# zombie-einstein/bourse

Hardware: AMD Instinct MI355X
Metric: book-steps/sec (higher is better)
Workload: dtype u32

## Files before the change

bourse_amd/csrc/event_asm.hpp:

```cpp
#pragma once
#include <hip/hip_runtime.h>
#include <stdint.h>

namespace bkd {

#define EA_BIT "s[40:41]"
#define EA_C0 "s[42:43]"
#define EA_C1 "s[44:45]"
#define EA_E0 "s[46:47]"
#define EA_E1 "s[48:49]"
#define EA_EW "s50"
#define EA_P "s51"
#define EA_V "s52"
#define EA_ID "s53"
#define EA_KK "s54"
#define EA_BEST "s55"
#define EA_PV "s56"
#define EA_PID "s57"
#define EA_TV "s58"
#define EA_LS "s59"
#define EA_X "s60"
#define EA_X2 "s61"

#define EA_IF2_1(x) ""
#define EA_IF2_2(x) x
#define EA_IF1_1(x) x
#define EA_IF1_2(x) ""

#define EA_DPP(OP)                                                                                \
  "s_nop 1\n\t" OP " %[vm], %[vm], %[vm] quad_perm:[1,0,3,2] row_mask:0xf bank_mask:0xf\n\t"      \
  "s_nop 1\n\t" OP " %[vm], %[vm], %[vm] quad_perm:[2,3,0,1] row_mask:0xf bank_mask:0xf\n\t"      \
  "s_nop 1\n\t" OP " %[vm], %[vm], %[vm] row_half_mirror row_mask:0xf bank_mask:0xf\n\t"          \
  "s_nop 1\n\t" OP " %[vm], %[vm], %[vm] row_mirror row_mask:0xf bank_mask:0xf\n\t"               \
  "s_nop 1\n\t" OP " %[vm], %[vm], %[vm] row_bcast:15 row_mask:0xa bank_mask:0xf\n\t"             \
  "s_nop 1\n\t" OP " %[vm], %[vm], %[vm] row_bcast:31 row_mask:0xc bank_mask:0xf\n\t"             \
  "s_nop 1\n\t"

#define EA_LOOP(PH, KEND)                       \
  "s_add_u32 %[k], %[k], 1\n\t"                 \
  "s_cmp_lt_u32 %[k], " KEND "\n\t"             \
  "s_cbranch_scc1 L_top_" PH "_%=\n\t"          \
  "s_branch L_end_" PH "_%=\n\t"

#define EA_PICK(Q, EQ, L)                                              \
  "s_ff1_i32_b64 " EA_LS ", " EQ "\n\t"                                \
  "v_readlane_b32 " EA_PV ", %[vol" Q "], " EA_LS "\n\t"               \
  "v_readlane_b32 " EA_PID ", %[id" Q "], " EA_LS "\n\t"               \
  "s_mov_b32 m0, " EA_LS "\n\t"                                        \
  "s_min_u32 " EA_TV ", " EA_V ", " EA_PV "\n\t"                       \
  "s_sub_u32 " EA_PV ", " EA_PV ", " EA_TV "\n\t"                      \
  "v_writelane_b32 %[vol" Q "], " EA_PV ", m0\n\t"                     \
  "s_cmp_lg_u32 " EA_PV ", 0\n\t"                                      \
  "s_cbranch_scc1 L_trade_" L "\n\t"                                   \
  "s_andn2_b64 %[live" Q "], %[live" Q "], " EQ "\n\t"

#ifndef BOURSE_AMD_ASM_ALWAYS_TIE
#define BOURSE_AMD_ASM_ALWAYS_TIE 0
#endif
#if BOURSE_AMD_ASM_ALWAYS_TIE
#define EA_TIE_TEST(L, NR) ""
#else
#define EA_TIE_TEST(L, NR)                                                                 \
  "s_bcnt1_i32_b64 " EA_X ", " EA_E0 "\n\t"                                                \
  EA_IF2_##NR("s_bcnt1_i32_b64 " EA_X2 ", " EA_E1 "\n\t"                                   \
              "s_add_u32 " EA_X ", " EA_X ", " EA_X2 "\n\t")                               \
  "s_cmp_eq_u32 " EA_X ", 1\n\t"                                                           \
  "s_cbranch_scc1 L_pick_" L "\n\t"
#endif

#define EA_SIDE(L, PH, KEND, RG, NR, CAND, SENT, VOP, DOP, NOX, KKI)                                     \
  KKI "\n\t"                                                                                        \
  "s_and_b32 " EA_X ", " EA_V ", %[tmask]\n\t"           \
  "s_cbranch_scc0 L_rest_" L "\n\t"                                                                 \
  "L_match_" L ":\n\t"                                                                              \
  CAND " " EA_C0 ", %[live0], %[bid0]\n\t"                      \
  EA_IF2_##NR(CAND " " EA_C1 ", %[live1], %[bid1]\n\t"                                              \
              "s_or_b64 " EA_E0 ", " EA_C0 ", " EA_C1 "\n\t")                                       \
  "s_cbranch_scc0 L_rest_" L "\n\t"                                   \
  "v_cndmask_b32_e64 %[vm], " SENT ", %[price0], " EA_C0 "\n\t"                                     \
  EA_IF2_##NR("v_cndmask_b32_e64 %[vm2], " SENT ", %[price1], " EA_C1 "\n\t"                        \
              VOP " %[vm], %[vm], %[vm2]\n\t")                                                      \
  EA_DPP(DOP)                                                                                       \
  "v_readlane_b32 " EA_BEST ", %[vm], 63\n\t"                                                       \
  NOX " " EA_P ", " EA_BEST "\n\t"                                                                  \
  "s_cbranch_scc1 L_rest_" L "\n\t"                                                                 \
  "v_cmp_eq_u32_e64 " EA_E0 ", " EA_BEST ", %[price0]\n\t"                                          \
  EA_IF2_##NR("v_cmp_eq_u32_e64 " EA_E1 ", " EA_BEST ", %[price1]\n\t")                             \
  "s_and_b64 " EA_E0 ", " EA_E0 ", " EA_C0 "\n\t"                                                   \
  EA_IF2_##NR("s_and_b64 " EA_E1 ", " EA_E1 ", " EA_C1 "\n\t")                                      \
  EA_TIE_TEST(L, NR)                                                                                \
   \
  "v_cndmask_b32_e64 %[vm], -1, %[seq0], " EA_E0 "\n\t"                                             \
  EA_IF2_##NR("v_cndmask_b32_e64 %[vm2], -1, %[seq1], " EA_E1 "\n\t"                                \
              "v_min_u32 %[vm], %[vm], %[vm2]\n\t")                                                 \
  EA_DPP("v_min_u32_dpp")                                                                           \
  "v_readlane_b32 " EA_X ", %[vm], 63\n\t"                                                          \
  "s_nop 1\n\t"                                                                                     \
  "v_cmp_eq_u32_e64 " EA_C0 ", " EA_X ", %[seq0]\n\t"                                               \
  EA_IF2_##NR("v_cmp_eq_u32_e64 " EA_C1 ", " EA_X ", %[seq1]\n\t")                                  \
  "s_and_b64 " EA_E0 ", " EA_E0 ", " EA_C0 "\n\t"                                                   \
  EA_IF2_##NR("s_and_b64 " EA_E1 ", " EA_E1 ", " EA_C1 "\n\t")                                      \
  "L_pick_" L ":\n\t"                                                                               \
  EA_IF2_##NR("s_cmp_lg_u64 " EA_E0 ", 0\n\t"                                                       \
              "s_cbranch_scc0 L_pick1_" L "\n\t")                                                   \
  EA_PICK("0", EA_E0, L)                                                                            \
  EA_IF2_##NR("s_branch L_trade_" L "\n\t"                                                          \
              "L_pick1_" L ":\n\t"                                                                  \
              EA_PICK("1", EA_E1, L))                                                               \
  "L_trade_" L ":\n\t"                                   \
  "s_sub_u32 " EA_V ", " EA_V ", " EA_TV "\n\t"                                                     \
  "s_add_u32 %[tvol], %[tvol], " EA_TV "\n\t"                                                       \
  "s_mov_b32 m0, %[trn]\n\t"                                                                        \
  "v_writelane_b32 %[trk], " EA_KK ", m0\n\t"                                                       \
  "v_writelane_b32 %[trp], " EA_BEST ", m0\n\t"                                                     \
  "v_writelane_b32 %[trv], " EA_TV ", m0\n\t"                                                       \
  "v_writelane_b32 %[tra], " EA_ID ", m0\n\t"                                                       \
  "v_writelane_b32 %[trs], " EA_PID ", m0\n\t"                                                      \
  "s_add_u32 %[trn], %[trn], 1\n\t"                                                                 \
  "s_cmp_eq_u32 %[trn], 64\n\t"                                                                     \
  "s_cbranch_scc1 L_full_" L "\n\t"                                                                 \
  "s_cmp_lg_u32 " EA_V ", 0\n\t"                                                                    \
  "s_cbranch_scc1 L_match_" L "\n\t"                                                                \
  EA_LOOP(PH, KEND)                                                      \
  "L_full_" L ":\n\t"                                               \
  "s_cmp_eq_u32 " EA_V ", 0\n\t"                                                                    \
  "s_cbranch_scc1 L_fullnext_%=\n\t"                                                                \
  "s_mov_b32 m0, " EA_EW "\n\t"                                                                     \
  "v_writelane_b32 %[vol" RG "], " EA_V ", m0\n\t"        \
  "s_branch L_flush_%=\n\t"                                                                         \
  "L_rest_" L ":\n\t"                                                                               \
  "s_cmp_eq_u32 " EA_P ", " SENT "\n\t"                   \
  "s_cbranch_scc1 L_next_" PH "_%=\n\t"                                                             \
  "s_mov_b32 m0, " EA_EW "\n\t"                                                                     \
  "v_writelane_b32 %[vol" RG "], " EA_V ", m0\n\t"                                                  \
  "v_writelane_b32 %[seq" RG "], %[seqc], m0\n\t"                                                   \
  "s_lshl_b64 " EA_BIT ", 1, " EA_EW "\n\t"                                                         \
  "s_or_b64 %[live" RG "], %[live" RG "], " EA_BIT "\n\t"                                           \
  "s_add_u32 %[seqc], %[seqc], 1\n\t"                                                               \
  EA_LOOP(PH, KEND)

#define EA_NEW(PH, KEND, RG, NR)                                                                          \
  "v_readlane_b32 " EA_P ", %[price" RG "], " EA_EW "\n\t"                                          \
  "v_readlane_b32 " EA_V ", %[vol" RG "], " EA_EW "\n\t"                                            \
  "v_readlane_b32 " EA_ID ", %[id" RG "], " EA_EW "\n\t"                                            \
  "s_bitcmp1_b32 " EA_EW ", 14\n\t"                                                                 \
  "s_cbranch_scc1 L_bid_" PH RG "_%=\n\t"                                                           \
  EA_SIDE("a" PH RG "_%=", PH, KEND, RG, NR, "s_and_b64", "0", "v_max_u32", "v_max_u32_dpp", "s_cmp_gt_u32", \
          "s_or_b32 " EA_KK ", %[k], 0x80000000")                                                   \
  "L_bid_" PH RG "_%=:\n\t"                                                                         \
  EA_SIDE("b" PH RG "_%=", PH, KEND, RG, NR, "s_andn2_b64", "-1", "v_min_u32", "v_min_u32_dpp", "s_cmp_lt_u32", \
          "s_mov_b32 " EA_KK ", %[k]")

#define EA_PHASE(PH, KEND, NR)                                                                      \
  "L_top_" PH "_%=:\n\t"                                                                            \
  "v_readlane_b32 " EA_EW ", %[ev" PH "], %[k]\n\t"                                                 \
  "s_bitcmp1_b32 " EA_EW ", 15\n\t"                                                                 \
  "s_cbranch_scc1 L_new_" PH "_%=\n\t"                                                              \
  "s_lshl_b64 " EA_BIT ", 1, " EA_EW "\n\t"                                       \
  EA_IF2_##NR("s_bitcmp1_b32 " EA_EW ", 6\n\t"                                                      \
              "s_cbranch_scc1 L_can1_" PH "_%=\n\t")                                                \
  "s_andn2_b64 %[live0], %[live0], " EA_BIT "\n\t"                                                  \
  EA_IF2_##NR(EA_LOOP(PH, KEND)                                                                     \
              "L_can1_" PH "_%=:\n\t"                                                               \
              "s_andn2_b64 %[live1], %[live1], " EA_BIT "\n\t")                                     \
  "L_next_" PH "_%=:\n\t"                                                                           \
  EA_LOOP(PH, KEND)                                                                                 \
  "L_new_" PH "_%=:\n\t"                                                                            \
  EA_IF2_##NR("s_bitcmp1_b32 " EA_EW ", 6\n\t"                                                      \
              "s_cbranch_scc1 L_new1_" PH "_%=\n\t")                                                \
  EA_IF1_##NR("s_nop 1\n\t")                                \
  EA_NEW(PH, KEND, "0", NR)                                                                               \
  EA_IF2_##NR("L_new1_" PH "_%=:\n\t"                                                               \
              EA_NEW(PH, KEND, "1", NR))

__device__ __forceinline__ uint32_t events_asm_r2(uint32_t& k, uint32_t n_ev, uint32_t tmask, uint32_t& tr_n,
                                                  uint32_t& seq_ctr, uint32_t& trade_vol, uint64_t& live0,
                                                  uint64_t& live1, uint64_t bid0, uint64_t bid1, uint32_t price0,
                                                  uint32_t price1, uint32_t& vol0, uint32_t& vol1, uint32_t id0,
                                                  uint32_t id1, uint32_t& seq0, uint32_t& seq1, uint32_t ev0,
                                                  uint32_t ev1, uint32_t& trk, uint32_t& trp, uint32_t& trv,
                                                  uint32_t& tra, uint32_t& trs) {
  uint32_t st, vm, vm2;
  auto u32 = [](uint32_t x) { return (uint32_t)__builtin_amdgcn_readfirstlane(x); };
  auto u64 = [&](uint64_t x) { return ((uint64_t)u32((uint32_t)(x >> 32)) << 32) | u32((uint32_t)x); };
  k = u32(k);
  n_ev = u32(n_ev);
  tmask = u32(tmask);
  tr_n = u32(tr_n);
  seq_ctr = u32(seq_ctr);
  trade_vol = u32(trade_vol);
  live0 = u64(live0);
  live1 = u64(live1);
  bid0 = u64(bid0);
  bid1 = u64(bid1);
  const uint32_t kend0 = n_ev < 64u ? n_ev : 64u;
  asm volatile(
      "s_cmp_lt_u32 %[k], %[kend0]\n\t"
      "s_cbranch_scc1 L_top_0_%=\n\t"
      "s_branch L_end_0_%=\n\t"
      EA_PHASE("0", "%[kend0]", 2)
      "L_end_0_%=:\n\t"
      "s_cmp_lt_u32 %[k], %[nev]\n\t"
      "s_cbranch_scc0 L_done_%=\n\t"
      EA_PHASE("1", "%[nev]", 2)
      "L_end_1_%=:\n\t"
      "L_done_%=:\n\t"
      "s_mov_b32 %[st], 0\n\t"
      "s_branch L_out_%=\n\t"
      "L_fullnext_%=:\n\t"
      "s_add_u32 %[k], %[k], 1\n\t"
      "L_flush_%=:\n\t"
      "s_mov_b32 %[st], 1\n\t"
      "L_out_%=:\n\t"
      "s_nop 1"
      : [st] "=&s"(st), [vm] "=&v"(vm), [vm2] "=&v"(vm2), [k] "+s"(k), [trn] "+s"(tr_n), [seqc] "+s"(seq_ctr),
        [tvol] "+s"(trade_vol), [live0] "+s"(live0), [live1] "+s"(live1), [vol0] "+v"(vol0), [vol1] "+v"(vol1),
        [seq0] "+v"(seq0), [seq1] "+v"(seq1), [trk] "+v"(trk), [trp] "+v"(trp), [trv] "+v"(trv), [tra] "+v"(tra),
        [trs] "+v"(trs)
      : [price0] "v"(price0), [price1] "v"(price1), [id0] "v"(id0), [id1] "v"(id1), [ev0] "v"(ev0), [ev1] "v"(ev1),
        [bid0] "s"(bid0), [bid1] "s"(bid1), [nev] "s"(n_ev), [kend0] "s"(kend0), [tmask] "s"(tmask)
      : "s40", "s41", "s42", "s43", "s44", "s45", "s46", "s47", "s48", "s49", "s50", "s51", "s52", "s53", "s54", "s55",
        "s56", "s57", "s58", "s59", "s60", "s61", "m0", "vcc", "scc", "memory");
  return st;
}

__device__ __forceinline__ uint32_t events_asm_r1(uint32_t& k, uint32_t n_ev, uint32_t tmask, uint32_t& tr_n,
                                                  uint32_t& seq_ctr, uint32_t& trade_vol, uint64_t& live0, uint64_t bid0,
                                                  uint32_t price0, uint32_t& vol0, uint32_t id0, uint32_t& seq0,
                                                  uint32_t ev0, uint32_t& trk, uint32_t& trp, uint32_t& trv,
                                                  uint32_t& tra, uint32_t& trs) {
  uint32_t st, vm;
  auto u32 = [](uint32_t x) { return (uint32_t)__builtin_amdgcn_readfirstlane(x); };
  auto u64 = [&](uint64_t x) { return ((uint64_t)u32((uint32_t)(x >> 32)) << 32) | u32((uint32_t)x); };
  k = u32(k);
  n_ev = u32(n_ev);
  tmask = u32(tmask);
  tr_n = u32(tr_n);
  seq_ctr = u32(seq_ctr);
  trade_vol = u32(trade_vol);
  live0 = u64(live0);
  bid0 = u64(bid0);
  asm volatile(
      "s_cmp_lt_u32 %[k], %[nev]\n\t"
      "s_cbranch_scc0 L_done_%=\n\t"
      EA_PHASE("0", "%[nev]", 1)
      "L_end_0_%=:\n\t"
      "L_done_%=:\n\t"
      "s_mov_b32 %[st], 0\n\t"
      "s_branch L_out_%=\n\t"
      "L_fullnext_%=:\n\t"
      "s_add_u32 %[k], %[k], 1\n\t"
      "L_flush_%=:\n\t"
      "s_mov_b32 %[st], 1\n\t"
      "L_out_%=:\n\t"
      "s_nop 1"
      : [st] "=&s"(st), [vm] "=&v"(vm), [k] "+s"(k), [trn] "+s"(tr_n), [seqc] "+s"(seq_ctr), [tvol] "+s"(trade_vol),
        [live0] "+s"(live0), [vol0] "+v"(vol0), [seq0] "+v"(seq0), [trk] "+v"(trk), [trp] "+v"(trp), [trv] "+v"(trv),
        [tra] "+v"(tra), [trs] "+v"(trs)
      : [price0] "v"(price0), [id0] "v"(id0), [ev0] "v"(ev0), [bid0] "s"(bid0), [nev] "s"(n_ev), [tmask] "s"(tmask)
      : "s40", "s41", "s42", "s43", "s44", "s45", "s46", "s47", "s48", "s49", "s50", "s51", "s52", "s53", "s54", "s55",
        "s56", "s57", "s58", "s59", "s60", "s61", "m0", "vcc", "scc", "memory");
  return st;
}

#define EK_KP EA_P
#define EK_ALO "s62"
#define EK_BHI "s63"

#define EK_PICK(Q, EQ, L, PH, KEND, SLOTI, SLOTW)                                                     \
  "s_ff1_i32_b64 " EA_LS ", " EQ "\n\t"                                                               \
  SLOTI                                                                                               \
  "s_mov_b32 m0, %[trn]\n\t"                                                                          \
  "v_readlane_b32 " EA_PV ", %[vol" Q "], " EA_LS "\n\t"                                              \
  "v_writelane_b32 %[trk], " EA_KK ", m0\n\t"                                                         \
  "v_writelane_b32 %[trs], " SLOTW ", m0\n\t"                                                         \
  "s_sub_u32 " EA_X ", " EA_PV ", " EA_V "\n\t"          \
  "s_cbranch_scc1 L_A" Q "_" L "\n\t"                                                                 \
  "v_writelane_b32 %[trv], " EA_V ", m0\n\t"             \
  "s_mov_b32 m0, " EA_LS "\n\t"                                                                       \
  "v_writelane_b32 %[vol" Q "], " EA_X ", m0\n\t"                                                     \
  "s_cmp_eq_u32 " EA_X ", 0\n\t"                                                                      \
  "s_cbranch_scc0 L_B" Q "_" L "\n\t"                                                                 \
  "v_writelane_b32 %[key" Q "], 0, m0\n\t"                     \
  "L_B" Q "_" L ":\n\t"                                                                               \
  "s_add_u32 %[trn], %[trn], 1\n\t"                                    \
  "s_cbranch_scc1 L_fullnext_%=\n\t"                                                                  \
  EA_LOOP(PH, KEND)                                                                                   \
  "L_A" Q "_" L ":\n\t"                                  \
  "v_writelane_b32 %[trv], " EA_PV ", m0\n\t"                                                         \
  "s_mov_b32 m0, " EA_LS "\n\t"                                                                       \
  "v_writelane_b32 %[vol" Q "], 0, m0\n\t"                                                            \
  "v_writelane_b32 %[key" Q "], 0, m0\n\t"                                                            \
  "s_sub_u32 " EA_V ", " EA_V ", " EA_PV "\n\t"                                                       \
  "s_add_u32 %[trn], %[trn], 1\n\t"                                                                   \
  "s_cbranch_scc1 L_fullA_" L "\n\t"                                                                  \
  "s_branch L_match_" L "\n\t"

#define EK_VCHK(L)                                   \
  "s_and_b32 " EA_X ", " EA_V ", %[tmask]\n\t"       \
  "s_cbranch_scc0 L_restq_" L "\n\t"
#define EK_VRD(RG) "v_readlane_b32 " EA_V ", %[vol" RG "], " EA_EW "\n\t"
#define EK_MKT(PH, KEND, L, MKTV)                                                                     \
  "s_cmp_eq_u32 " EK_KP ", " MKTV "\n\t"                                                              \
  "s_cbranch_scc0 L_dorest_" L "\n\t"                                                                \
  EA_LOOP(PH, KEND)                                                                                   \
  "L_dorest_" L ":\n\t"
#define EK_SIDE(L, PH, KEND, RG, NR, KPI, VOP, DOP, NOX, KKI, OPPB, SKIP, OWNB, PULL, VCHK, VLATE, MK) \
  KPI "\n\t"                                                                                          \
  VCHK                                                                                                \
  SKIP " " EK_KP ", " OPPB "\n\t"                                 \
  "s_cbranch_scc1 L_restq_" L "\n\t"                                                                  \
  VLATE                                                                                               \
  KKI "\n\t"                                                     \
  "L_match_" L ":\n\t"                                                                                \
  EA_IF1_##NR("v_mov_b32 %[vm], %[key0]\n\t")                                                         \
  EA_IF2_##NR(VOP " %[vm], %[key0], %[key1]\n\t")                                                     \
  EA_DPP(DOP)                                                                                         \
  "v_readlane_b32 " OPPB ", %[vm], 63\n\t"              \
  "s_nop 1\n\t"                                             \
                               \
  "v_cmp_eq_u32_e64 " EA_E0 ", " OPPB ", %[key0]\n\t"                                                 \
  EA_IF2_##NR("v_cmp_eq_u32_e64 " EA_E1 ", " OPPB ", %[key1]\n\t")                                    \
  NOX " " OPPB ", " EK_KP "\n\t"                                                                      \
  "s_cbranch_scc1 L_rest_" L "\n\t"                                                                   \
  EA_IF2_##NR("s_cmp_lg_u64 " EA_E0 ", 0\n\t"                                                         \
              "s_cbranch_scc0 L_pick1_" L "\n\t")                                                     \
  EK_PICK("0", EA_E0, L, PH, KEND, "", EA_LS)                                                         \
  EA_IF2_##NR("L_pick1_" L ":\n\t"                                                                    \
              EK_PICK("1", EA_E1, L, PH, KEND, "s_or_b32 " EA_PID ", " EA_LS ", 64\n\t", EA_PID))        \
  "L_fullA_" L ":\n\t"                                   \
  "s_mov_b32 m0, " EA_EW "\n\t"                                                                       \
  "v_writelane_b32 %[vol" RG "], " EA_V ", m0\n\t"                                                    \
  "s_branch L_flush_%=\n\t"                                                                           \
  "L_rest_" L ":\n\t"                                        \
  "s_mov_b32 m0, " EA_EW "\n\t"                                                                       \
  "v_writelane_b32 %[vol" RG "], " EA_V ", m0\n\t"                                                    \
  "L_restq_" L ":\n\t"                                                          \
  MK                                                                                                  \
  "s_mov_b32 m0, " EA_EW "\n\t"                                                                       \
  "s_xor_b32 " EA_X ", " EK_KP ", %[sq]\n\t"                                                          \
  PULL " " OWNB ", " OWNB ", " EA_X "\n\t"               \
  "v_writelane_b32 %[key" RG "], " EA_X ", m0\n\t"                                                    \
  "s_add_u32 %[sq], %[sq], 1\n\t"                                                                     \
  EA_LOOP(PH, KEND)

#define EK_NOMK(PH, KEND, L, MKTV) ""
#define EK_NEW(PH, KEND, RG, NR, CHK, VE, VL, MKM)                                                    \
  VE(EK_VRD(RG))                                                                                      \
  "s_bitcmp1_b32 " EA_EW ", 14\n\t"                                                                   \
  "s_cbranch_scc1 L_bid_" PH RG "_%=\n\t"                                                             \
   \
  EK_SIDE("a" PH RG "_%=", PH, KEND, RG, NR, "s_and_b32 " EK_KP ", " EA_EW ", 0xffff0000", "v_max_i32", "v_max_i32_dpp", \
          "s_cmp_lt_i32", "s_or_b32 " EA_KK ", %[k], 0x80000000", EK_BHI, "s_cmp_gt_i32", EK_ALO, "s_min_i32", \
          CHK("a" PH RG "_%="), VL(EK_VRD(RG)), MKM(PH, KEND, "a" PH RG "_%=", "0x10000"))             \
  "L_bid_" PH RG "_%=:\n\t"                                                                           \
  EK_SIDE("b" PH RG "_%=", PH, KEND, RG, NR, "s_or_b32 " EK_KP ", " EA_EW ", 0xffff", "v_min_i32", "v_min_i32_dpp", \
          "s_cmp_gt_i32", "s_mov_b32 " EA_KK ", %[k]", EK_ALO, "s_cmp_lt_i32", EK_BHI, "s_max_i32", CHK("b" PH RG "_%="), \
          VL(EK_VRD(RG)), MKM(PH, KEND, "b" PH RG "_%=", "-1"))

#define EK_NOCHK(L) ""
#define EK_ID(x) x
#define EK_NONE(x) ""
#define EK_PHASE(PH, EVN, KEND, NR, CHK, VE, VL) EK_PHASE_M(PH, EVN, KEND, NR, CHK, VE, VL, EK_NOMK)
#define EK_PHASE_M(PH, EVN, KEND, NR, CHK, VE, VL, MKM)                                               \
  "L_top_" PH "_%=:\n\t"                                                                              \
  "v_readlane_b32 " EA_EW ", %[ev" EVN "], %[k]\n\t"                                                  \
  "s_bitcmp1_b32 " EA_EW ", 15\n\t"                                                                   \
  "s_cbranch_scc1 L_new_" PH "_%=\n\t"                                                                \
                                                                          \
  EA_IF2_##NR("s_bitcmp1_b32 " EA_EW ", 6\n\t"                                                        \
              "s_cbranch_scc1 L_can1_" PH "_%=\n\t")                                                  \
  EA_IF1_##NR("s_nop 1\n\t")                                                                          \
  "v_writelane_b32 %[key0], 0, " EA_EW "\n\t"                                                         \
  EA_IF2_##NR(EA_LOOP(PH, KEND)                                                                       \
              "L_can1_" PH "_%=:\n\t"                                                                 \
              "v_writelane_b32 %[key1], 0, " EA_EW "\n\t")                                            \
  EA_LOOP(PH, KEND)                                                                                   \
  "L_new_" PH "_%=:\n\t"                                                                              \
  EA_IF2_##NR("s_bitcmp1_b32 " EA_EW ", 6\n\t"                                                        \
              "s_cbranch_scc1 L_new1_" PH "_%=\n\t")                                                  \
  EA_IF1_##NR("s_nop 1\n\t")                                  \
  EK_NEW(PH, KEND, "0", NR, CHK, VE, VL, MKM)                                                         \
  EA_IF2_##NR("L_new1_" PH "_%=:\n\t"                                                                 \
              EK_NEW(PH, KEND, "1", NR, CHK, VE, VL, MKM))

#define EK_TAIL                     \
  "L_done_%=:\n\t"                  \
  "s_mov_b32 %[st], 0\n\t"          \
  "s_branch L_out_%=\n\t"           \
  "L_fullnext_%=:\n\t"              \
  "s_add_u32 %[k], %[k], 1\n\t"     \
  "L_flush_%=:\n\t"                 \
  "s_mov_b32 %[st], 1\n\t"          \
  "L_out_%=:\n\t"                   \
  "s_nop 1"

#define EK_CLOBBERS                                                                                                 \
  "s40", "s41", "s42", "s43", "s44", "s45", "s46", "s47", "s48", "s49", "s50", "s51", "s52", "s53", "s54", "s55",  \
      "s56", "s57", "s58", "s59", "s60", "s61", "s62", "s63", "m0", "vcc", "scc", "memory"

#define EK_BINIT "s_mov_b32 " EK_ALO ", 0x80000000\n\t" "s_mov_b32 " EK_BHI ", 0x7fffffff\n\t"
#define EK_NOBOPS
#define EK_R2_STMT_X(MKM, BINIT, BOPS) \
  asm volatile( \
      BINIT \
      "s_cmp_eq_u32 %[chk], 0\n\t" \
      "s_cbranch_scc1 L_fast_%=\n\t" \
      "s_cmp_lt_u32 %[k], %[kend0]\n\t" \
      "s_cbranch_scc1 L_top_0_%=\n\t" \
      "s_branch L_end_0_%=\n\t" \
      EK_PHASE_M("0", "0", "%[kend0]", 2, EK_VCHK, EK_ID, EK_NONE, MKM) \
      "L_end_0_%=:\n\t" \
      "s_cmp_lt_u32 %[k], %[nev]\n\t" \
      "s_cbranch_scc0 L_done_%=\n\t" \
      EK_PHASE_M("1", "1", "%[nev]", 2, EK_VCHK, EK_ID, EK_NONE, MKM) \
      "L_end_1_%=:\n\t" \
      "s_branch L_done_%=\n\t" \
      "L_fast_%=:\n\t" \
      "s_cmp_lt_u32 %[k], %[kend0]\n\t" \
      "s_cbranch_scc1 L_top_2_%=\n\t" \
      "s_branch L_end_2_%=\n\t" \
      EK_PHASE_M("2", "0", "%[kend0]", 2, EK_NOCHK, EK_NONE, EK_ID, MKM) \
      "L_end_2_%=:\n\t" \
      "s_cmp_lt_u32 %[k], %[nev]\n\t" \
      "s_cbranch_scc0 L_done_%=\n\t" \
      EK_PHASE_M("3", "1", "%[nev]", 2, EK_NOCHK, EK_NONE, EK_ID, MKM) \
      "L_end_3_%=:\n\t" \
      EK_TAIL \
      : [st] "=&s"(st), [vm] "=&v"(vm), [k] "+s"(k), [trn] "+s"(trn), [sq] "+s"(sq), \
        [vol0] "+v"(vol0), [vol1] "+v"(vol1), [key0] "+v"(key0), \
        [key1] "+v"(key1), [trk] "+v"(trk), [trv] "+v"(trv), [trs] "+v"(trs) BOPS \
      : [ev0] "v"(ev0), [ev1] "v"(ev1), \
        [nev] "s"(n_ev), [kend0] "s"(kend0), [tmask] "s"(tmask), [chk] "s"(checked) \
      : EK_CLOBBERS);

#define EK_R1_STMT_X(MKM, BINIT, BOPS) \
  asm volatile( \
      BINIT \
      "s_cmp_lt_u32 %[k], %[nev]\n\t" \
      "s_cbranch_scc0 L_done_%=\n\t" \
      "s_cmp_eq_u32 %[chk], 0\n\t" \
      "s_cbranch_scc1 L_top_2_%=\n\t" \
      EK_PHASE_M("0", "0", "%[nev]", 1, EK_VCHK, EK_ID, EK_NONE, MKM) \
      "L_end_0_%=:\n\t" \
      "s_branch L_done_%=\n\t" \
      EK_PHASE_M("2", "0", "%[nev]", 1, EK_NOCHK, EK_NONE, EK_ID, MKM) \
      "L_end_2_%=:\n\t" \
      EK_TAIL \
      : [st] "=&s"(st), [vm] "=&v"(vm), [k] "+s"(k), [trn] "+s"(trn), [sq] "+s"(sq), \
        [vol0] "+v"(vol0), [key0] "+v"(key0), [trk] "+v"(trk), [trv] "+v"(trv), [trs] "+v"(trs) BOPS \
      : [ev0] "v"(ev0), [nev] "s"(n_ev), [tmask] "s"(tmask), [chk] "s"(checked) \
      : EK_CLOBBERS);

#define EK_R2_STMT EK_R2_STMT_X(EK_NOMK, EK_BINIT, EK_NOBOPS)
#define EK_R1_STMT EK_R1_STMT_X(EK_NOMK, EK_BINIT, EK_NOBOPS)
#define EK_BOPS , [alo] "+s"(alo), [bhi] "+s"(bhi)
#define EK_R2M_STMT EK_R2_STMT_X(EK_MKT, "", EK_BOPS)
#define EK_R1M_STMT EK_R1_STMT_X(EK_MKT, "", EK_BOPS)

__device__ __forceinline__ uint32_t events_key_r2(uint32_t checked, uint32_t& k, uint32_t n_ev, uint32_t tmask, uint32_t& tr_n, uint32_t& sq,
                                                  uint32_t& vol0, uint32_t& vol1, uint32_t& key0, uint32_t& key1, uint32_t ev0,
                                                  uint32_t ev1, uint32_t& trk, uint32_t& trv, uint32_t& trs) {
  uint32_t st, vm;
  auto u32 = [](uint32_t x) { return (uint32_t)__builtin_amdgcn_readfirstlane(x); };
  checked = u32(checked);
  k = u32(k);
  n_ev = u32(n_ev);
  tmask = u32(tmask);
  uint32_t trn = u32(tr_n) - 64u;
  sq = u32(sq);
  const uint32_t kend0 = n_ev < 64u ? n_ev : 64u;
  EK_R2_STMT
  tr_n = trn + 64u;
  return st;
}

__device__ __forceinline__ uint32_t events_key_r1(uint32_t checked, uint32_t& k, uint32_t n_ev, uint32_t tmask, uint32_t& tr_n, uint32_t& sq,
                                                  uint32_t& vol0, uint32_t& key0, uint32_t ev0, uint32_t& trk, uint32_t& trv,
                                                  uint32_t& trs) {
  uint32_t st, vm;
  auto u32 = [](uint32_t x) { return (uint32_t)__builtin_amdgcn_readfirstlane(x); };
  checked = u32(checked);
  k = u32(k);
  n_ev = u32(n_ev);
  tmask = u32(tmask);
  uint32_t trn = u32(tr_n) - 64u;
  sq = u32(sq);
  EK_R1_STMT
  tr_n = trn + 64u;
  return st;
}

#undef EK_ALO
#undef EK_BHI
#define EK_ALO "%[alo]"
#define EK_BHI "%[bhi]"
__device__ __forceinline__ uint32_t events_key_r2m(uint32_t checked, uint32_t& k, uint32_t n_ev, uint32_t tmask, uint32_t& tr_n, uint32_t& sq,
                                                   uint32_t& vol0, uint32_t& vol1, uint32_t& key0, uint32_t& key1, uint32_t ev0,
                                                   uint32_t ev1, uint32_t& trk, uint32_t& trv, uint32_t& trs, uint32_t& alo,
                                                   uint32_t& bhi) {
  uint32_t st, vm;
  alo = (uint32_t)__builtin_amdgcn_readfirstlane(alo);
  bhi = (uint32_t)__builtin_amdgcn_readfirstlane(bhi);
  auto u32 = [](uint32_t x) { return (uint32_t)__builtin_amdgcn_readfirstlane(x); };
  checked = u32(checked);
  k = u32(k);
  n_ev = u32(n_ev);
  tmask = u32(tmask);
  uint32_t trn = u32(tr_n) - 64u;
  sq = u32(sq);
  const uint32_t kend0 = n_ev < 64u ? n_ev : 64u;
  EK_R2M_STMT
  tr_n = trn + 64u;
  return st;
}

__device__ __forceinline__ uint32_t events_key_r1m(uint32_t checked, uint32_t& k, uint32_t n_ev, uint32_t tmask, uint32_t& tr_n, uint32_t& sq,
                                                   uint32_t& vol0, uint32_t& key0, uint32_t ev0, uint32_t& trk, uint32_t& trv,
                                                   uint32_t& trs, uint32_t& alo, uint32_t& bhi) {
  uint32_t st, vm;
  alo = (uint32_t)__builtin_amdgcn_readfirstlane(alo);
  bhi = (uint32_t)__builtin_amdgcn_readfirstlane(bhi);
  auto u32 = [](uint32_t x) { return (uint32_t)__builtin_amdgcn_readfirstlane(x); };
  checked = u32(checked);
  k = u32(k);
  n_ev = u32(n_ev);
  tmask = u32(tmask);
  uint32_t trn = u32(tr_n) - 64u;
  sq = u32(sq);
  EK_R1M_STMT
  tr_n = trn + 64u;
  return st;
}

}
```

Before: 309.9 million.

## Bias loop counter negative so increment sets loop-exit flag, rotating event lanes

The inner event loops now run the counter k as a negative offset relative to the phase end. The add that increments it sets the carry flag at the end, which replaces the separate compare per iteration. To keep lane indexing consistent, event registers are rotated with ds_bpermute on entry and ds_permute back on exit, and k is restored in the tail paths. This saves a scalar compare per event but adds LDS permute round-trips per call, and it makes ev0 and ev1 in-out operands.

```diff
diff --git a/bourse_amd/csrc/event_asm.hpp b/bourse_amd/csrc/event_asm.hpp
--- a/bourse_amd/csrc/event_asm.hpp
+++ b/bourse_amd/csrc/event_asm.hpp
@@ -266,6 +266,37 @@
 #define EK_KP EA_P
 #define EK_ALO "s62"
 #define EK_BHI "s63"
+#define EK_KOFS "s53"
+#define EK_LOOP(PH)                     \
+  "s_add_u32 %[k], %[k], 1\n\t"         \
+  "s_cbranch_scc0 L_top_" PH "_%=\n\t"  \
+  "s_branch L_end_" PH "_%=\n\t"
+#define EK_ENTER(PH, KEND)                              \
+  "s_sub_u32 %[k], %[k], " KEND "\n\t"                  \
+  "s_cbranch_scc0 L_end_" PH "_%=\n\t"                  \
+  "s_or_b32 " EK_KOFS ", " KEND ", 0x80000000\n\t"
+#define EK_ROT(OP, EV, KEND)                             \
+  "v_mbcnt_lo_u32_b32 %[vm], -1, 0\n\t"                   \
+  "v_mbcnt_hi_u32_b32 %[vm], -1, %[vm]\n\t"               \
+  "v_add_lshl_u32 %[vm], %[vm], " KEND ", 2\n\t"          \
+  "v_and_b32 %[vm], 0xfc, %[vm]\n\t"                      \
+  OP " %[" EV "], %[vm], %[" EV "]\n\t"
+#define EK_ROT_IN_R2                                     \
+  "s_nop 1\n\t"                                          \
+  EK_ROT("ds_bpermute_b32", "ev0", "%[kend0]")            \
+  EK_ROT("ds_bpermute_b32", "ev1", "%[nev]")              \
+  "s_waitcnt lgkmcnt(0)\n\t"
+#define EK_ROT_OUT_R2                                    \
+  EK_ROT("ds_permute_b32", "ev0", "%[kend0]")             \
+  EK_ROT("ds_permute_b32", "ev1", "%[nev]")               \
+  "s_waitcnt lgkmcnt(0)\n\t"
+#define EK_ROT_IN_R1                                     \
+  "s_nop 1\n\t"                                          \
+  EK_ROT("ds_bpermute_b32", "ev0", "%[nev]")              \
+  "s_waitcnt lgkmcnt(0)\n\t"
+#define EK_ROT_OUT_R1                                    \
+  EK_ROT("ds_permute_b32", "ev0", "%[nev]")               \
+  "s_waitcnt lgkmcnt(0)\n\t"
 
 #define EK_PICK(Q, EQ, L, PH, KEND, SLOTI, SLOTW)                                                     \
   "s_ff1_i32_b64 " EA_LS ", " EQ "\n\t"                                                               \
@@ -285,7 +316,7 @@
   "L_B" Q "_" L ":\n\t"                                                                               \
   "s_add_u32 %[trn], %[trn], 1\n\t"                                    \
   "s_cbranch_scc1 L_fullnext_%=\n\t"                                                                  \
-  EA_LOOP(PH, KEND)                                                                                   \
+  EK_LOOP(PH)                                                                                         \
   "L_A" Q "_" L ":\n\t"                                  \
   "v_writelane_b32 %[trv], " EA_PV ", m0\n\t"                                                         \
   "s_mov_b32 m0, " EA_LS "\n\t"                                                                       \
@@ -303,7 +334,7 @@
 #define EK_MKT(PH, KEND, L, MKTV)                                                                     \
   "s_cmp_eq_u32 " EK_KP ", " MKTV "\n\t"                                                              \
   "s_cbranch_scc0 L_dorest_" L "\n\t"                                                                \
-  EA_LOOP(PH, KEND)                                                                                   \
+  EK_LOOP(PH)                                                                                         \
   "L_dorest_" L ":\n\t"
 #define EK_SIDE(L, PH, KEND, RG, NR, KPI, VOP, DOP, NOX, KKI, OPPB, SKIP, OWNB, PULL, VCHK, VLATE, MK) \
   KPI "\n\t"                                                                                          \
@@ -342,7 +373,7 @@
   PULL " " OWNB ", " OWNB ", " EA_X "\n\t"               \
   "v_writelane_b32 %[key" RG "], " EA_X ", m0\n\t"                                                    \
   "s_add_u32 %[sq], %[sq], 1\n\t"                                                                     \
-  EA_LOOP(PH, KEND)
+  EK_LOOP(PH)
 
 #define EK_NOMK(PH, KEND, L, MKTV) ""
 #define EK_NEW(PH, KEND, RG, NR, CHK, VE, VL, MKM)                                                    \
@@ -351,11 +382,11 @@
   "s_cbranch_scc1 L_bid_" PH RG "_%=\n\t"                                                             \
    \
   EK_SIDE("a" PH RG "_%=", PH, KEND, RG, NR, "s_and_b32 " EK_KP ", " EA_EW ", 0xffff0000", "v_max_i32", "v_max_i32_dpp", \
-          "s_cmp_lt_i32", "s_or_b32 " EA_KK ", %[k], 0x80000000", EK_BHI, "s_cmp_gt_i32", EK_ALO, "s_min_i32", \
+          "s_cmp_lt_i32", "s_add_u32 " EA_KK ", %[k], " EK_KOFS, EK_BHI, "s_cmp_gt_i32", EK_ALO, "s_min_i32",   \
           CHK("a" PH RG "_%="), VL(EK_VRD(RG)), MKM(PH, KEND, "a" PH RG "_%=", "0x10000"))             \
   "L_bid_" PH RG "_%=:\n\t"                                                                           \
   EK_SIDE("b" PH RG "_%=", PH, KEND, RG, NR, "s_or_b32 " EK_KP ", " EA_EW ", 0xffff", "v_min_i32", "v_min_i32_dpp", \
-          "s_cmp_gt_i32", "s_mov_b32 " EA_KK ", %[k]", EK_ALO, "s_cmp_lt_i32", EK_BHI, "s_max_i32", CHK("b" PH RG "_%="), \
+          "s_cmp_gt_i32", "s_add_u32 " EA_KK ", %[k], " KEND, EK_ALO, "s_cmp_lt_i32", EK_BHI, "s_max_i32", CHK("b" PH RG "_%="), \
           VL(EK_VRD(RG)), MKM(PH, KEND, "b" PH RG "_%=", "-1"))
 
 #define EK_NOCHK(L) ""
@@ -372,10 +403,10 @@
               "s_cbranch_scc1 L_can1_" PH "_%=\n\t")                                                  \
   EA_IF1_##NR("s_nop 1\n\t")                                                                          \
   "v_writelane_b32 %[key0], 0, " EA_EW "\n\t"                                                         \
-  EA_IF2_##NR(EA_LOOP(PH, KEND)                                                                       \
+  EA_IF2_##NR(EK_LOOP(PH)                                                                             \
               "L_can1_" PH "_%=:\n\t"                                                                 \
               "v_writelane_b32 %[key1], 0, " EA_EW "\n\t")                                            \
-  EA_LOOP(PH, KEND)                                                                                   \
+  EK_LOOP(PH)                                                                                         \
   "L_new_" PH "_%=:\n\t"                                                                              \
   EA_IF2_##NR("s_bitcmp1_b32 " EA_EW ", 6\n\t"                                                        \
               "s_cbranch_scc1 L_new1_" PH "_%=\n\t")                                                  \
@@ -384,15 +415,19 @@
   EA_IF2_##NR("L_new1_" PH "_%=:\n\t"                                                                 \
               EK_NEW(PH, KEND, "1", NR, CHK, VE, VL, MKM))
 
-#define EK_TAIL                     \
-  "L_done_%=:\n\t"                  \
-  "s_mov_b32 %[st], 0\n\t"          \
-  "s_branch L_out_%=\n\t"           \
-  "L_fullnext_%=:\n\t"              \
-  "s_add_u32 %[k], %[k], 1\n\t"     \
-  "L_flush_%=:\n\t"                 \
-  "s_mov_b32 %[st], 1\n\t"          \
-  "L_out_%=:\n\t"                   \
+#define EK_TAIL(ROT_OUT)                         \
+  "L_done_%=:\n\t"                               \
+  "s_add_u32 %[k], %[k], %[nev]\n\t"             \
+  "s_mov_b32 %[st], 0\n\t"                       \
+  "s_branch L_out_%=\n\t"                        \
+  "L_fullnext_%=:\n\t"                           \
+  "s_add_u32 %[k], %[k], 1\n\t"                  \
+  "L_flush_%=:\n\t"                              \
+  "s_add_u32 %[k], %[k], " EK_KOFS "\n\t"        \
+  "s_bitset0_b32 %[k], 31\n\t"                   \
+  "s_mov_b32 %[st], 1\n\t"                       \
+  "L_out_%=:\n\t"                                \
+  ROT_OUT                                        \
   "s_nop 1"
 
 #define EK_CLOBBERS                                                                                                 \
@@ -404,41 +439,37 @@
 #define EK_R2_STMT_X(MKM, BINIT, BOPS) \
   asm volatile( \
       BINIT \
+      EK_ROT_IN_R2 \
       "s_cmp_eq_u32 %[chk], 0\n\t" \
       "s_cbranch_scc1 L_fast_%=\n\t" \
-      "s_cmp_lt_u32 %[k], %[kend0]\n\t" \
-      "s_cbranch_scc1 L_top_0_%=\n\t" \
-      "s_branch L_end_0_%=\n\t" \
+      EK_ENTER("0", "%[kend0]") \
       EK_PHASE_M("0", "0", "%[kend0]", 2, EK_VCHK, EK_ID, EK_NONE, MKM) \
       "L_end_0_%=:\n\t" \
-      "s_cmp_lt_u32 %[k], %[nev]\n\t" \
-      "s_cbranch_scc0 L_done_%=\n\t" \
+      "s_add_u32 %[k], %[k], %[kend0]\n\t" \
+      EK_ENTER("1", "%[nev]") \
       EK_PHASE_M("1", "1", "%[nev]", 2, EK_VCHK, EK_ID, EK_NONE, MKM) \
       "L_end_1_%=:\n\t" \
       "s_branch L_done_%=\n\t" \
       "L_fast_%=:\n\t" \
-      "s_cmp_lt_u32 %[k], %[kend0]\n\t" \
-      "s_cbranch_scc1 L_top_2_%=\n\t" \
-      "s_branch L_end_2_%=\n\t" \
+      EK_ENTER("2", "%[kend0]") \
       EK_PHASE_M("2", "0", "%[kend0]", 2, EK_NOCHK, EK_NONE, EK_ID, MKM) \
       "L_end_2_%=:\n\t" \
-      "s_cmp_lt_u32 %[k], %[nev]\n\t" \
-      "s_cbranch_scc0 L_done_%=\n\t" \
+      "s_add_u32 %[k], %[k], %[kend0]\n\t" \
+      EK_ENTER("3", "%[nev]") \
       EK_PHASE_M("3", "1", "%[nev]", 2, EK_NOCHK, EK_NONE, EK_ID, MKM) \
       "L_end_3_%=:\n\t" \
-      EK_TAIL \
+      EK_TAIL(EK_ROT_OUT_R2) \
       : [st] "=&s"(st), [vm] "=&v"(vm), [k] "+s"(k), [trn] "+s"(trn), [sq] "+s"(sq), \
         [vol0] "+v"(vol0), [vol1] "+v"(vol1), [key0] "+v"(key0), \
-        [key1] "+v"(key1), [trk] "+v"(trk), [trv] "+v"(trv), [trs] "+v"(trs) BOPS \
-      : [ev0] "v"(ev0), [ev1] "v"(ev1), \
-        [nev] "s"(n_ev), [kend0] "s"(kend0), [tmask] "s"(tmask), [chk] "s"(checked) \
+        [key1] "+v"(key1), [trk] "+v"(trk), [trv] "+v"(trv), [trs] "+v"(trs), [ev0] "+v"(ev0), [ev1] "+v"(ev1) BOPS \
+      : [nev] "s"(n_ev), [kend0] "s"(kend0), [tmask] "s"(tmask), [chk] "s"(checked) \
       : EK_CLOBBERS);
 
 #define EK_R1_STMT_X(MKM, BINIT, BOPS) \
   asm volatile( \
       BINIT \
-      "s_cmp_lt_u32 %[k], %[nev]\n\t" \
-      "s_cbranch_scc0 L_done_%=\n\t" \
+      EK_ROT_IN_R1 \
+      EK_ENTER("0", "%[nev]") \
       "s_cmp_eq_u32 %[chk], 0\n\t" \
       "s_cbranch_scc1 L_top_2_%=\n\t" \
       EK_PHASE_M("0", "0", "%[nev]", 1, EK_VCHK, EK_ID, EK_NONE, MKM) \
@@ -446,10 +477,10 @@
       "s_branch L_done_%=\n\t" \
       EK_PHASE_M("2", "0", "%[nev]", 1, EK_NOCHK, EK_NONE, EK_ID, MKM) \
       "L_end_2_%=:\n\t" \
-      EK_TAIL \
+      EK_TAIL(EK_ROT_OUT_R1) \
       : [st] "=&s"(st), [vm] "=&v"(vm), [k] "+s"(k), [trn] "+s"(trn), [sq] "+s"(sq), \
-        [vol0] "+v"(vol0), [key0] "+v"(key0), [trk] "+v"(trk), [trv] "+v"(trv), [trs] "+v"(trs) BOPS \
-      : [ev0] "v"(ev0), [nev] "s"(n_ev), [tmask] "s"(tmask), [chk] "s"(checked) \
+        [vol0] "+v"(vol0), [key0] "+v"(key0), [trk] "+v"(trk), [trv] "+v"(trv), [trs] "+v"(trs), [ev0] "+v"(ev0) BOPS \
+      : [nev] "s"(n_ev), [tmask] "s"(tmask), [chk] "s"(checked) \
       : EK_CLOBBERS);
 
 #define EK_R2_STMT EK_R2_STMT_X(EK_NOMK, EK_BINIT, EK_NOBOPS)
@@ -459,8 +490,8 @@
 #define EK_R1M_STMT EK_R1_STMT_X(EK_MKT, "", EK_BOPS)
 
 __device__ __forceinline__ uint32_t events_key_r2(uint32_t checked, uint32_t& k, uint32_t n_ev, uint32_t tmask, uint32_t& tr_n, uint32_t& sq,
-                                                  uint32_t& vol0, uint32_t& vol1, uint32_t& key0, uint32_t& key1, uint32_t ev0,
-                                                  uint32_t ev1, uint32_t& trk, uint32_t& trv, uint32_t& trs) {
+                                                  uint32_t& vol0, uint32_t& vol1, uint32_t& key0, uint32_t& key1, uint32_t& ev0,
+                                                  uint32_t& ev1, uint32_t& trk, uint32_t& trv, uint32_t& trs) {
   uint32_t st, vm;
   auto u32 = [](uint32_t x) { return (uint32_t)__builtin_amdgcn_readfirstlane(x); };
   checked = u32(checked);
@@ -476,7 +507,7 @@
 }
 
 __device__ __forceinline__ uint32_t events_key_r1(uint32_t checked, uint32_t& k, uint32_t n_ev, uint32_t tmask, uint32_t& tr_n, uint32_t& sq,
-                                                  uint32_t& vol0, uint32_t& key0, uint32_t ev0, uint32_t& trk, uint32_t& trv,
+                                                  uint32_t& vol0, uint32_t& key0, uint32_t& ev0, uint32_t& trk, uint32_t& trv,
                                                   uint32_t& trs) {
   uint32_t st, vm;
   auto u32 = [](uint32_t x) { return (uint32_t)__builtin_amdgcn_readfirstlane(x); };
@@ -496,8 +527,8 @@
 #define EK_ALO "%[alo]"
 #define EK_BHI "%[bhi]"
 __device__ __forceinline__ uint32_t events_key_r2m(uint32_t checked, uint32_t& k, uint32_t n_ev, uint32_t tmask, uint32_t& tr_n, uint32_t& sq,
-                                                   uint32_t& vol0, uint32_t& vol1, uint32_t& key0, uint32_t& key1, uint32_t ev0,
-                                                   uint32_t ev1, uint32_t& trk, uint32_t& trv, uint32_t& trs, uint32_t& alo,
+                                                   uint32_t& vol0, uint32_t& vol1, uint32_t& key0, uint32_t& key1, uint32_t& ev0,
+                                                   uint32_t& ev1, uint32_t& trk, uint32_t& trv, uint32_t& trs, uint32_t& alo,
                                                    uint32_t& bhi) {
   uint32_t st, vm;
   alo = (uint32_t)__builtin_amdgcn_readfirstlane(alo);
@@ -516,7 +547,7 @@
 }
 
 __device__ __forceinline__ uint32_t events_key_r1m(uint32_t checked, uint32_t& k, uint32_t n_ev, uint32_t tmask, uint32_t& tr_n, uint32_t& sq,
-                                                   uint32_t& vol0, uint32_t& key0, uint32_t ev0, uint32_t& trk, uint32_t& trv,
+                                                   uint32_t& vol0, uint32_t& key0, uint32_t& ev0, uint32_t& trk, uint32_t& trv,
                                                    uint32_t& trs, uint32_t& alo, uint32_t& bhi) {
   uint32_t st, vm;
   alo = (uint32_t)__builtin_amdgcn_readfirstlane(alo);
```

Result: no change. 310.6 million (median of 6 runs) (+0.2%).
